# qwerty35/lsc_dr_planner

Hardware: AMD Instinct MI355X
Metric: qp_solves_per_sec (higher is better)
Workload: dtype f64; 1 GPU; configs[1]: 64 agents x M=5 x ~20 LSC half-spaces/seg, fp64 -- 64 agents/GPU x M=5 segments x 20 LSC neighbours (dim=3, forest swarm after 3 warm-up replans), fp64: dual active-set phase (one workgroup per QP) with the batched PDIP behind it for what it leaves; batch_seed=1000, precision=f64, row_format=f64, collective_backend=none (single process), agents_per_gpu=64, agents_total=64, ranks=1, distinct_devices=1, launch=single process, segments=5, lsc_neighbours=20, dim=3, rows_per_qp=1074, allgather=False, pipeline=False, hip_graph=False

## Files before the change

lsc_dr_planner_amd/csrc/lscqp_das_body.inc:

```
#if LSCQP_DAS_PROLOGUE
#define DAS_CLS(f) ka_##f
#else
#define DAS_CLS(f) cls.f
#endif
    const int tid = threadIdx.x, lane = tid & 63, wv = tid >> 6;
#ifdef LSCQP_DAS_LAYOUT
    constexpr Layout L = LSCQP_DAS_LAYOUT;
#else
    const Layout L = Layout::make(M, dim, kmax, cacheC, stage_rows);
#endif
    DAS_T_DECL();
    const int P = L.P, NX = L.NX, NPAIR = L.NPAIR;
    const int kcap = L.kmax;
    double* const H_ = smem + L.o_hdr;
    double* const sfc_ = smem + L.o_sfc;
    double* const c_ = smem + L.o_c;
    double* const cu_ = smem + L.o_cu;
    double* const lam_ = smem + L.o_lam;
    double* const plo_ = smem + L.o_plo;
    double* const phi_ = smem + L.o_phi;
    int* const pix_ = reinterpret_cast<int*>(smem + L.o_pix);
    double* const W_ = smem + L.o_W;
    double* const Jm_ = smem + L.o_L;
    double* const u_ = smem + L.o_u;
// ... 81 lines not shown
    int2 pwr[kPB];
#pragma unroll
    for (int u = 0; u < kPB; u++) pwr[u] = pairs_g[min(tid + u * T, NPAIR - 1)];
    {
        const double* hsrc = reinterpret_cast<const double*>(hdr + q);
        const double* ssrc = reinterpret_cast<const double*>(sfc) + q * 6 * M;
        for (int e = tid; e < 32 + (cls.use_sfc ? 6 * M : 0); e += T) (e < 32 ? H_[e] : sfc_[e - 32]) = e < 32 ? hsrc[e] : ssrc[e - 32];
        if (tid >= 64 - 36 && tid < 64) dq_[tid - (64 - 36)] = tab[(size_t)M * table_stride(M) + (tid - (64 - 36))];
        if (tid < 6) {
            const double w = tid == 0 ? cls.world_min[0] : tid == 1 ? cls.world_min[1] : tid == 2 ? cls.world_min[2] : tid == 3 ? cls.world_max[0] : tid == 4 ? cls.world_max[1] : cls.world_max[2];
            wb_[tid] = w;
        }
    }
    __syncthreads();
#endif
    DAS_T(0);
    const lscqp_header* Hd = reinterpret_cast<const lscqp_header*>(H_);
    const lscqp_box* sfcl = reinterpret_cast<const lscqp_box*>(sfc_);
#if !LSCQP_DAS_PROLOGUE
    const int n_obs = Hd->n_obs;
#endif
    auto hand_over = [&](int steps, int why) {
        for (int e = tid; e < NX; e += T) x_out[q * NX + e] = x_init ? x_init[q * NX + e] : Hd->p0[fdiv(e, 1.0f / (float)P)];
        if (tid == 0) {
            obj_out[q] = 0.0;
            status_out[q] = LSCQP_STATUS_ITER_LIMIT;
            if (info_out) {
                info_out[q].iterations = 0;
                info_out[q].flags = 0;
                info_out[q].res_primal = 0.0;
                info_out[q].res_dual = (double)why;
                info_out[q].gap = (double)steps;
            }
        }
    };
    auto infeasible_out = [&](int steps, double violation) {
        for (int e = tid; e < NX; e += T) x_out[q * NX + e] = x_init ? x_init[q * NX + e] : Hd->p0[fdiv(e, 1.0f / (float)P)];
        if (tid == 0) {
            obj_out[q] = 0.0;
            status_out[q] = LSCQP_STATUS_INFEASIBLE;
            if (info_out) {
                info_out[q].iterations = steps;
                info_out[q].flags = LSCQP_INFO_ACTIVE_SET;
                info_out[q].res_primal = violation;
                info_out[q].res_dual = 0.0;
                info_out[q].gap = 0.0;
            }
        }
    };
#if LSCQP_DAS_PROLOGUE
    if (!in_cap)
#else
    if (n_obs > cap || n_obs < 0)
#endif
    {
        hand_over(0, LSCQP_DAS_WHY_CAPACITY);
        LSCQP_DAS_END(kDasHandedOver);
    }
    const double dt = DAS_CLS(dt);
    const double org0 = Hd->p0[0], org1 = Hd->p0[1], org2 = Hd->p0[2];
    const double* const org = Hd->p0;
    int ts = Hd->terminal_segments;
    if (ts <= 0) {
        const double g0 = Hd->goal[0] - org0, g1 = Hd->goal[1] - org1, g2 = Hd->goal[2] - org2;
        ts = (int)((M * dt - sqrt(g0 * g0 + g1 * g1 + g2 * g2) / Hd->nominal_velocity + 1e-9) / dt);
        if (ts < 1) ts = 1;
    }
    if (ts > M) ts = M;
    const double q2s = DAS_CLS(q2s), wt2 = 2.0 * DAS_CLS(w_t);
    const double* const tb = tab + (size_t)(ts - 1) * table_stride(M);
    const double* const U1 = tb, * const U2 = tb + P, * const G1 = tb + 2 * P, * const Cg = tb + 3 * P;
    const bool comm_on = DAS_CLS(comm_range) > 0;
    const double rho_pair = 0.5 * DAS_CLS(comm_range) - Hd->radius;
    const double rho_wp = 0.5 * DAS_CLS(comm_range) - 1e-5;
#if !LSCQP_DAS_PROLOGUE
    const int nL = n_obs * P;
#endif
    const float iP = 1.0f / (float)P;
    const bool staged = stage_rows > 0 && nL <= stage_rows;
    bool rows_in_lds = false;

#if LSCQP_DAS_PROLOGUE
    constexpr int NE = 4;
    double tu1[NE], tu2[NE], tg1[NE];
#pragma unroll
    for (int i = 0; i < NE; i++) {
        const int e = tid + i * T < NX ? tid + i * T : 0;
        const int cp = e - P * fdiv(e, iP);
        tu1[i] = U1[cp], tu2[i] = U2[cp], tg1[i] = G1[cp];
    }
#else
    auto fetch_row = [&](int j, double& x, double& y, double& z, double& w) {
        if constexpr (F32) {
            const float4 f = reinterpret_cast<const float4*>(rows)[roff + (uint64_t)j];
            x = f.x, y = f.y, z = f.z, w = f.w;
        } else {
            const double4 d = *reinterpret_cast<const double4*>(&rows[roff + (uint64_t)j]);
            x = d.x, y = d.y, z = d.z, w = d.w;
        }
    };
    constexpr int NE = 4;
    double tu1[NE], tu2[NE], tg1[NE];
#pragma unroll
    for (int i = 0; i < NE; i++) {
        const int e = tid + i * T;
        if (e < NX) {
            const int cp = e - P * fdiv(e, iP);
            tu1[i] = U1[cp], tu2[i] = U2[cp], tg1[i] = G1[cp];
        }
    }
    double px[kU], py[kU], pz[kU], pw[kU];
#pragma unroll
    for (int u = 0; u < kU; u++) px[u] = py[u] = pz[u] = 0.0, pw[u] = -1.0;
    if (nL > 0) {
#pragma unroll
        for (int u = 0; u < kU; u++) {
            const int j = tid + u * T;
            fetch_row(j < nL ? j : 0, px[u], py[u], pz[u], pw[u]);
        }
    }
#endif

    constexpr int kCPre = (NW == 4 && !PEEL && !SCREEN) ? 6 : 0;
    double cpre[kCPre > 0 ? kCPre : 1];
#if LSCQP_DAS_PROLOGUE
    const bool c_fits = kCPre > 0 && P * P <= kCPre * T;
    const bool c_prefetched = c_fits && cacheC;
#else
    const bool c_prefetched = kCPre > 0 && cacheC && P * P <= kCPre * T;
    const bool c_fits = c_prefetched;
#endif
    if constexpr (kCPre > 0) {
        if (c_fits) {
#pragma unroll
            for (int i = 0; i < kCPre; i++) {
                const int e = tid + i * T;
                cpre[i] = Cg[e < P * P ? e : 0];
            }
        }
    }
#if LSCQP_DAS_STEP_PATH & 2
#ifndef LSCQP_DAS_LAYOUT
#error "LSCQP_DAS_STEP_PATH & 2 needs the compile-time carve"
#endif
    static_assert(NW > 1, "the first pass's barrier publishes the table");
    constexpr bool kTableEarly = kCPre > 0 && L.P * L.P <= kCPre * T;
    static_assert(!kTableEarly || LSCQP_DAS_PROLOGUE, "the table is stored from cpre[]: it needs the prologue that always loads it");
#else
    constexpr bool kTableEarly = false;
#endif

    bool empty = false;
    const double hv_c = dt * 0.2, ha_c = dt * dt * 0.05;
    for (int r0 = tid; r0 < NPAIR; r0 += kPB * T) {
        if (r0 != tid) {
#pragma unroll
            for (int u = 0; u < kPB; u++) pwr[u] = pairs_g[min(r0 + u * T, NPAIR - 1)];
        }
#pragma unroll
        for (int u = 0; u < kPB; u++) {
            if ((r0 - tid) + u * T >= NPAIR) break;
            const int r = r0 + u * T;
            const int w0 = pwr[u].x, w1 = pwr[u].y;
            const int fam = w1 & 3, k = (w1 >> 2) & 3, m = (w1 >> 4) & 15;
            const bool last = (w1 >> 8) & 1, rs = (w1 >> 9) & 1;
            const double ok_ = org[k], wlo = wb_[k], whi = wb_[3 + k], wpk = Hd->next_waypoint[k] - ok_;
            const double hv = Hd->vmax[k] * hv_c, ha = Hd->amax[k] * ha_c;
            double lo = wlo - ok_, hi = whi - ok_;
            if (DAS_CLS(rsfc) && rs) {
                lo = -100.0 - ok_;
                hi = 100.0 - ok_;
            }
            if (DAS_CLS(use_sfc)) {
                lo = fmax(lo, sfcl[m].bmin[k] - ok_);
                hi = fmin(hi, sfcl[m].bmax[k] - ok_);
            }
            const double clo = fmax(lo, fmax(-rho_pair, wpk - rho_wp)), chi = fmin(hi, fmin(rho_pair, wpk + rho_wp));
            lo = (comm_on && last) ? clo : lo;
            hi = (comm_on && last) ? chi : hi;
            const double hs = fam == 1 ? hv : fam == 2 ? ha : rho_pair;
            lo = fam == 0 ? lo : -hs;
            hi = fam == 0 ? hi : hs;
            if (r < NPAIR) {
                if (fam == 0 && (w0 >> 24) != 0 && lo > hi) empty = true;
                plo_[r] = lo, phi_[r] = hi;
                pix_[r] = w0;
            }
        }
    }
#pragma unroll
    for (int i = 0; i < NE; i++) {
        const int e = tid + i * T;
        if (e < NX) {
            const int k = fdiv(e, iP), cp = e - k * P;
            const double c1 = Hd->v0[k] * dt * 0.2;
            const double c2 = Hd->a0[k] * dt * dt * 0.05 + 2.0 * c1;
            const double fixv = (cp == 1) ? c1 : (cp == 2) ? c2 : 0.0;
            const double cv = fixv - c1 * tu1[i] - c2 * tu2[i] + wt2 * (Hd->goal[k] - org[k]) * tg1[i];
            c_[e] = cv;
            cu_[e] = cv;
        }
    }
    if (dim == 2)
        for (int e = tid; e < P; e += T) c_[2 * P + e] = 0.0;
#if LSCQP_DAS_STEP_PATH & 2
    {
        double2* const J2 = reinterpret_cast<double2*>(Jm_);
        for (int e = tid; e < kcap * LDL / 2; e += T) J2[e] = make_double2(0.0, 0.0);
    }
#endif
#if LSCQP_DAS_STEP_PATH & 8
    for (int e = tid; e < NX; e += T) lam_[e] = 0.0;
#endif
#if LSCQP_DAS_PROLOGUE
    const bool empty_w = __ballot(empty) != 0;
    if constexpr (NW > 1) {
        if (lane == 0) red_[20 + wv] = empty_w ? 1.0 : 0.0;
    }
    LSCQP_DAS_BARRIER();
    bool empty_g = empty_w;
    if constexpr (NW > 1) {
        empty_g = false;
#pragma unroll
        for (int w = 0; w < NW; w++) empty_g = empty_g || red_[20 + w] != 0.0;
    }
#else
    if (tid == 0) ctl_[4] = 0.0;
    LSCQP_DAS_BARRIER();
    if (empty) ctl_[4] = 1.0;
    LSCQP_DAS_BARRIER();
#endif
#if LSCQP_DAS_PROLOGUE
    if (empty_g)
#else
    if (ctl_[4] != 0.0)
#endif
    {
        double ov = 0.0;
        if (wv == 0) {
            for (int r = lane; r < NPAIR; r += 64)
                if ((pix_[r] >> 24) != 0) ov = fmax(ov, plo_[r] - phi_[r]);
            ov = wave_max(ov);
        }
        infeasible_out(0, ov);
        LSCQP_DAS_END(kDasInfeasible);
    }
    DAS_T(1);

    auto translate = [&](int j, double x, double y, double z, double w, double& nx, double& ny, double& nz, double& b) -> bool {
        nx = x, ny = y, nz = (dim == 3) ? z : 0.0;
        b = (dim == 3) ? w - (x * org0 + y * org1 + z * org2) : w - (x * org0 + y * org1 + 0.0);
        return !(x * x + y * y + z * z < 1e-10) && (j - P * fdiv(j, iP)) >= 3;
    };
    auto load_row = [&](int j, double& nx, double& ny, double& nz, double& b) -> bool {
        if (rows_in_lds) {
            nx = Sx_[j], ny = Sy_[j], nz = Sz_[j], b = Sb_[j];
            return b != -1.0 || nx != 0.0 || ny != 0.0 || nz != 0.0;
        }
        double x, y, z, w;
        fetch_row(j, x, y, z, w);
        return translate(j, x, y, z, w, nx, ny, nz, b);
    };
    auto pair_val = [&](int pk, const double* vec) -> double {
        const int type = pk >> 24, e0 = (pk >> 12) & 0xfff, e1 = pk & 0xfff;
        const int i0 = (type == 4) ? e1 : e0 + max(type - 1, 0);
        const int i1 = (type == 3) ? e0 + 1 : e0;
        const double a1 = (type <= 1) ? 0.0 : (type == 3) ? -2.0 : -1.0;
        const double a2 = (type == 3) ? 1.0 : 0.0;
        const double v0 = vec[i0], v1 = vec[i1], v2 = vec[e0];
        return (v0 + a1 * v1) + a2 * v2;
    };
    auto ent_of = [&](int e) -> int {
        const int k = fdiv(e, iP);
        return (k << 16) | (e - k * P);
    };
    auto decode = [&](int rid, Row& R) {
        R.ent[0] = R.ent[1] = R.ent[2] = 0;
        R.coef[0] = R.coef[1] = R.coef[2] = 0.0;
        if (rid < nL) {
            const int cp = rid - P * fdiv(rid, iP);
            double nx, ny, nz, b;
            (void)load_row(rid, nx, ny, nz, b);
            R.ent[0] = cp, R.ent[1] = (1 << 16) | cp, R.ent[2] = (2 << 16) | cp;
            R.coef[0] = nx, R.coef[1] = ny, R.coef[2] = (dim == 3) ? nz : 0.0;
            R.rhs = b;
            return;
        }
        const int s = rid - nL, r = s >> 1, pk = pix_[r];
        const int type = pk >> 24, e0 = (pk >> 12) & 0xfff, e1 = pk & 0xfff;
        const double sg = (s & 1) ? -1.0 : 1.0;
        R.rhs = (s & 1) ? -phi_[r] : plo_[r];
        const bool t1 = type == 1, t2 = type == 2, t3 = type == 3;
        R.ent[0] = ent_of(t1 ? e0 : t2 ? e0 + 1 : t3 ? e0 + 2 : e1);
        R.ent[1] = t1 ? 0 : ent_of(t3 ? e0 + 1 : e0);
        R.ent[2] = t3 ? ent_of(e0) : 0;
        R.coef[0] = sg;
        R.coef[1] = t1 ? 0.0 : t3 ? -2.0 * sg : -sg;
        R.coef[2] = t3 ? sg : 0.0;
    };
    auto row_dot = [&](const int* ent, const double* coef, const double* vec) -> double {
        return coef[0] * vec[ent_axis(ent[0]) * P + ent_cp(ent[0])] + coef[1] * vec[ent_axis(ent[1]) * P + ent_cp(ent[1])] +
               coef[2] * vec[ent_axis(ent[2]) * P + ent_cp(ent[2])];
    };

    bool first_pass = true;
    auto pass_local = [&](double& bv, int& bi) {
        bv = 1e300;
        bi = 0x7fffffff;
        auto see = [&](double slack, int id) {
            slack = (slack == slack) ? slack : -1e308;
            const bool lt = slack < bv;
            bv = lt ? slack : bv;
            bi = lt ? id : bi;
        };
        auto eval = [&](int j0, const double* rx, const double* ry, const double* rz, const double* rb) {
#pragma unroll
            for (int u = 0; u < kU; u++) {
                const int j = j0 + u * T, jc = j < nL ? j : 0;
                const int cp = jc - P * fdiv(jc, iP);
                see(rx[u] * c_[cp] + ry[u] * c_[P + cp] + rz[u] * c_[2 * P + cp] - rb[u], j);
            }
        };
        auto prep = [&](int j0, const double* x, const double* y, const double* z, const double* w, double* rx, double* ry, double* rz, double* rb) {
#pragma unroll
            for (int u = 0; u < kU; u++) {
                const int j = j0 + u * T, jc = j < nL ? j : 0;
                const bool ok = translate(jc, x[u], y[u], z[u], w[u], rx[u], ry[u], rz[u], rb[u]) && j < nL;
                rx[u] = ok ? rx[u] : 0.0, ry[u] = ok ? ry[u] : 0.0, rz[u] = ok ? rz[u] : 0.0, rb[u] = ok ? rb[u] : -1.0;
            }
        };
        auto stage = [&](int j0, const double* rx, const double* ry, const double* rz, const double* rb) {
#pragma unroll
            for (int u = 0; u < kU; u++) {
                const int j = j0 + u * T;
                if (j < nL) Sx_[j] = rx[u], Sy_[j] = ry[u], Sz_[j] = rz[u], Sb_[j] = rb[u];
            }
        };
        double rx[kU], ry[kU], rz[kU], rb[kU];
        if (first_pass) {
            prep(tid, px, py, pz, pw, rx, ry, rz, rb);
            if (staged) stage(tid, rx, ry, rz, rb);
            eval(tid, rx, ry, rz, rb);
            for (int j0 = tid + kU * T; kMaxNL > kU * T && j0 < nL; j0 += kU * T) {
                double x[kU], y[kU], z[kU], w[kU];
#pragma unroll
                for (int u = 0; u < kU; u++) fetch_row(j0 + u * T < nL ? j0 + u * T : 0, x[u], y[u], z[u], w[u]);
                prep(j0, x, y, z, w, rx, ry, rz, rb);
                if (staged) stage(j0, rx, ry, rz, rb);
                eval(j0, rx, ry, rz, rb);
            }
        } else if (rows_in_lds) {
#if LSCQP_DAS_STEP_PATH & 1
            for (int j0 = tid; j0 < nL; j0 += kU * T) {
                double lx[kU], ly[kU], lz[kU], lb[kU];
#pragma unroll
                for (int u = 0; u < kU; u++) {
                    const int j = j0 + u * T, jc = j < nL ? j : 0;
                    lx[u] = Sx_[jc], ly[u] = Sy_[jc], lz[u] = Sz_[jc], lb[u] = Sb_[jc];
                }
#pragma unroll
                for (int u = 0; u < kU; u++) {
                    const bool in = j0 + u * T < nL;
                    rx[u] = in ? lx[u] : 0.0, ry[u] = in ? ly[u] : 0.0, rz[u] = in ? lz[u] : 0.0, rb[u] = in ? lb[u] : -1.0;
                }
                eval(j0, rx, ry, rz, rb);
            }
#else
            for (int j0 = tid; j0 < nL; j0 += kU * T) {
#pragma unroll
                for (int u = 0; u < kU; u++) {
                    const int j = j0 + u * T, jc = j < nL ? j : 0;
                    rx[u] = Sx_[jc], ry[u] = Sy_[jc], rz[u] = Sz_[jc], rb[u] = (j < nL) ? Sb_[jc] : 1e300;
                    if (!(j < nL)) rx[u] = ry[u] = rz[u] = 0.0, rb[u] = -1.0;
                }
                eval(j0, rx, ry, rz, rb);
            }
#endif
        } else {
            for (int j0 = tid; j0 < nL; j0 += kU * T) {
                double x[kU], y[kU], z[kU], w[kU];
#pragma unroll
                for (int u = 0; u < kU; u++) fetch_row(j0 + u * T < nL ? j0 + u * T : 0, x[u], y[u], z[u], w[u]);
                prep(j0, x, y, z, w, rx, ry, rz, rb);
                eval(j0, rx, ry, rz, rb);
            }
        }
        first_pass = false;
        DAS_T(8);
        for (int r0 = tid; r0 < NPAIR; r0 += 2 * T) {
            const int r1 = r0 + T, r1c = r1 < NPAIR ? r1 : r0;
            const int pk0 = pix_[r0], pk1 = pix_[r1c];
            const double lo0 = plo_[r0], hi0 = phi_[r0], lo1 = plo_[r1c], hi1 = phi_[r1c];
            const double d0 = pair_val(pk0, c_), d1 = pair_val(pk1, c_);
            const bool on0 = (pk0 >> 24) != 0, on1 = (pk1 >> 24) != 0 && r1 < NPAIR;
            see(on0 ? d0 - lo0 : 1.0, nL + 2 * r0);
            see(on0 ? hi0 - d0 : 1.0, nL + 2 * r0 + 1);
            see(on1 ? d1 - lo1 : 1.0, nL + 2 * r1);
            see(on1 ? hi1 - d1 : 1.0, nL + 2 * r1 + 1);
        }
        DAS_T(9);
    };
    auto pass_combine = [&](const double* rb_, double& bv, int& bi) {
        bv = rb_[0], bi = reinterpret_cast<const int*>(rb_ + 4)[0];
#pragma unroll
        for (int w = 1; w < NW; w++) {
            const double ov = rb_[w];
            const int oi = reinterpret_cast<const int*>(rb_ + 4)[w];
            if (ov < bv || (ov == bv && oi < bi)) bv = ov, bi = oi;
        }
    };
    auto pass = [&](double& best, int& bid) {
        const bool was_first = first_pass;
        double bv;
        int bi;
        pass_local(bv, bi);
#if LSCQP_DAS_STEP_PATH & 2
        if constexpr (kTableEarly) {
            if (was_first) {
#pragma unroll
                for (int i = 0; i < kCPre; i++) {
                    const int e = tid + i * T;
                    if (e < P * P) Cc_[e] = cpre[i];
                }
            }
        }
#endif
        wave_argmin(bv, bi);
        if constexpr (NW > 1) {
            double* const rb_ = red_ + 24 * par;
            par ^= 1;
            if (lane == 0) {
                rb_[wv] = bv;
                reinterpret_cast<int*>(rb_ + 4)[wv] = bi;
            }
            LSCQP_DAS_BARRIER();
            pass_combine(rb_, bv, bi);
        } else if (staged && was_first) {
            LSCQP_DAS_BARRIER();
        }
        if (staged) rows_in_lds = true;
        best = bv, bid = bi;
    };

    const double* Cm = kTableEarly ? Cc_ : Cg;
    auto factor_remove = [&](int k_, int l_) -> bool {
        bool ok = true;
        if (wv == 0) {
            const int k = __builtin_amdgcn_readfirstlane(k_), l = __builtin_amdgcn_readfirstlane(l_);
            const bool mine = lane < k;
            const int c = mine ? lane : 0;
            const int cn = c - (c > l ? 1 : 0);
            double carry = Jm_[l * LDL + c];
            double a = Jm_[l * LDL + l];
            for (int j = l; j < k - 1; j++) {
                const double x = Jm_[(j + 1) * LDL + c];
                const double b = Jm_[(j + 1) * LDL + l];
                const double r2 = a * a + b * b;
                if (!(r2 > 1e-280)) ok = false;
                const double ir = rsqrt(fmax(r2, 1e-300));
                const double ca = a * ir, sb = b * ir;
                const double fin = ca * x - sb * carry;
                carry = ca * carry + sb * x;
                a = r2 * ir;
                if (mine && lane != l) Jm_[j * LDL + cn] = fin;
            }
            if (mine) Jm_[(k - 1) * LDL + lane] = 0.0, Jm_[lane * LDL + k - 1] = 0.0;
            LSCQP_DAS_WAVE_SYNC();
        }
        return ok;
    };
    auto solve_factor = [&](int k_, double vi, double* yy) -> double {
        const int k = __builtin_amdgcn_readfirstlane(k_);
        const bool mine = lane < k;
        const int ll = min(lane, kcap - 1);
        vi = mine ? vi : 0.0;
        double yi = 0.0, ri = 0.0;
        for (int j0 = 0; j0 < k; j0 += 8) {
            double Jr[8];
#pragma unroll
            for (int t_ = 0; t_ < 8; t_++) Jr[t_] = Jm_[ll * LDL + min(j0 + t_, kcap)];
#pragma unroll
            for (int t_ = 0; t_ < 8; t_++) yi += Jr[t_] * lscqp::bcast(vi, j0 + t_);
        }
        yi = mine ? yi : 0.0;
        if (yy) *yy = wave_sum(yi * yi);
        for (int j0 = 0; j0 < k; j0 += 8) {
            double Jc[8];
#pragma unroll
            for (int t_ = 0; t_ < 8; t_++) Jc[t_] = Jm_[min(j0 + t_, kcap - 1) * LDL + ll];
#pragma unroll
            for (int t_ = 0; t_ < 8; t_++) ri += Jc[t_] * lscqp::bcast(yi, j0 + t_);
        }
        ri = mine ? ri : 0.0;
        if (lane < kcap + 4) r_[lane] = ri;
        return ri;
    };
    auto add_columns = [&](int k, const double* wts, const double* base) {
        for (int e = tid; e < NX; e += T) {
            double a = base ? base[e] : c_[e];
            for (int j = 0; j < k; j++) a += wts[j] * W_[(size_t)j * NX + e];
            c_[e] = a;
        }
    };

    const int NZA = 3 * (M - 1) + (es ? 1 : 3);
    auto finish_local = [&](int k, double& rd, double& gs, double& part) {
#if LSCQP_DAS_PROLOGUE
        const double dt = wb_[6], q2s = wb_[7], ka_w_t = ctl_[4], ka_w_c = red_[44], wt2 = 2.0 * ka_w_t;
#endif
#if LSCQP_DAS_STEP_PATH & 8
#if !LSCQP_DAS_PROLOGUE
#error "LSCQP_DAS_STEP_PATH & 8 reads the class's scalars from LDS: it needs the rescheduled prologue"
#endif
        static_assert(NW > 1, "the stationarity rows take one trip of the workgroup");
        auto objective_local = [&]() {
#if LSCQP_DAS_STEP_PATH & 32
            static_assert(NW > 1, "the objective's lanes are the second wavefront's");
            part = 0.0;
            if (__builtin_amdgcn_readfirstlane(wv) == 1) {
                const bool on = lane < dim * M;
                const int lv = on ? lane : dim * M - 1;
                const int kx = lv / M, m = lv - kx * M;
                const double* cc = &c_[kx * P + 6 * m];
                double cv[6], dqv[36];
                double ok_ = org[kx], gl_ = Hd->goal[kx];
#pragma unroll
                for (int i = 0; i < 6; i++) cv[i] = cc[i];
#pragma unroll
                for (int i = 0; i < 36; i++) dqv[i] = dq_[i];
                asm volatile("" : "+v"(ok_), "+v"(gl_));
#pragma unroll
                for (int i = 0; i < 6; i++) asm volatile("" : "+v"(cv[i]));
#pragma unroll
                for (int i = 0; i < 36; i++) asm volatile("" : "+v"(dqv[i]));
                const double j0 = (cv[3] - cv[0]) - 3.0 * (cv[2] - cv[1]);
                const double j1 = (cv[4] - cv[1]) - 3.0 * (cv[3] - cv[2]);
                const double j2 = (cv[5] - cv[2]) - 3.0 * (cv[4] - cv[3]);
                const double quad = 0.2 * (j0 * j0 + j2 * j2) + (2.0 / 15.0) * j1 * j1 + 0.2 * (j0 * j1 + j1 * j2) + (1.0 / 15.0) * j0 * j2;
                double pp = 0.5 * q2s * 3600.0 * quad;
                double corr = 0;
                const double s0 = cv[0] + ok_, s1 = cv[1] + ok_, s2 = cv[2] + ok_, s3 = cv[3] + ok_, s4 = cv[4] + ok_, s5 = cv[5] + ok_;
#pragma unroll
                for (int i = 0; i < 6; i++) {
                    const double* dr = dqv + 6 * i;
                    double r = 0;
                    r += dr[0] * s0, r += dr[1] * s1, r += dr[2] * s2, r += dr[3] * s3, r += dr[4] * s4, r += dr[5] * s5;
                    corr += r * (cv[i] + ok_);
                }
                pp += DAS_CLS(w_c) * corr;
                const double dgoal = cv[5] - (gl_ - ok_);
                pp += (m >= M - ts) ? DAS_CLS(w_t) * dgoal * dgoal : 0.0;
                const double sum = part + pp;
                part = on ? sum : part;
            }
#else
            part = 0.0;
            for (int lv = tid - (NW > 1 ? 64 : 0); lv < dim * M; lv += T) {
                if (lv < 0) continue;
                const int kx = lv / M, m = lv - kx * M;
                const double* cc = &c_[kx * P + 6 * m];
                const double j0 = (cc[3] - cc[0]) - 3.0 * (cc[2] - cc[1]);
                const double j1 = (cc[4] - cc[1]) - 3.0 * (cc[3] - cc[2]);
// ... 182 lines not shown
        for (int w = 1; w < NW; w++) rd = fmax(rd, rb_[8 + w]), gs = fmax(gs, rb_[12 + w]), part += rb_[16 + w];
    };
    auto finish_verdict = [&](double rd, double gs, double part, double& res_d, double& obj) {
        res_d = (part == part && fabs(part) < 1e300) ? rd / fmax(1.0, gs) : 1e300;
        obj = part;
    };
    auto finish = [&](int k, double& res_d, double& obj) {
        double rd, gs, part;
        finish_local(k, rd, gs, part);
        lscqp::wave_reduce3<lscqp::OpMax, lscqp::OpMax, lscqp::OpSum>(rd, gs, part);
        if constexpr (NW > 1) {
            double* const rb_ = red_ + 24 * par;
            par ^= 1;
            if (lane == 0) rb_[8 + wv] = rd, rb_[12 + wv] = gs, rb_[16 + wv] = part;
            LSCQP_DAS_BARRIER();
            finish_combine(rb_, rd, gs, part);
        }
        finish_verdict(rd, gs, part, res_d, obj);
    };

    int k = 0, steps = 0, why = LSCQP_DAS_WHY_VERIFICATION;
    bool polished = false, solved = false, haveC = false, haveJ = false, proven = false;
    double res_p = 0.0, res_d = 0.0, obj = 0.0;
    auto write_out = [&]() {
        for (int e = tid; e < NX; e += T) x_out[q * NX + e] = c_[e] + org[fdiv(e, iP)];
        if (tid == 0) {
            obj_out[q] = obj;
            status_out[q] = LSCQP_STATUS_OPTIMAL;
            if (info_out) {
                info_out[q].iterations = steps;
                info_out[q].flags = LSCQP_INFO_ACTIVE_SET;
                info_out[q].res_primal = res_p;
                info_out[q].res_dual = res_d;
                info_out[q].gap = 0.0;
            }
        }
    };
    double best;
    int bid;
    bool peeled = false;
    if constexpr (PEEL || SCREEN) {
        pass(best, bid);
        DAS_T(2);
        if (!(best < -kTolP)) {
            res_p = fmax(0.0, -best);
            finish(0, res_d, obj);
            DAS_T(4);
            if (res_d <= kTolD) write_out();
            else hand_over(0, LSCQP_DAS_WHY_VERIFICATION);
            DAS_T(7);
            DAS_T_FLUSH();
            LSCQP_DAS_END(res_d <= kTolD ? kDasSolved : kDasHandedOver);
        }
        peeled = true;
    }
    for (;;) {
        if (!((PEEL || SCREEN) && peeled)) {
            pass(best, bid);
            DAS_T(steps == 0 ? 2 : 3);
        }
        peeled = false;
        if (!(best < -kTolP)) {
            res_p = fmax(0.0, -best);
            finish(k, res_d, obj);
            DAS_T(4);
            if (res_d <= kTolD) {
                solved = true;
                break;
            }
            if (polished || k == 0) break;
#if LSCQP_DAS_STEP_PATH & 8
            if (tid == 0) {
                for (int j_ = 0; j_ < k; j_++)
#pragma unroll
                    for (int t_ = 0; t_ < 3; t_++) {
                        const int en = aint_[4 * j_ + 1 + t_], at = ent_axis(en) * P + ent_cp(en);
                        if (at < NX) lam_[at] = 0.0;
                    }
            }
#endif
            LSCQP_DAS_BARRIER();
            add_columns(k, u_, cu_);
            LSCQP_DAS_BARRIER();
            if (wv == 0) {
                const double rho = (lane < k) ? arhs_[lane] - row_dot(&aint_[4 * lane + 1], &acoef_[3 * lane], c_) : 0.0;
                const double du = solve_factor(k, rho, nullptr);
                const double un = (lane < k) ? u_[lane] + du : 0.0;
                const double umax = wave_max(fabs(un));
                const double neg = wave_max((lane < k && un < -1e-12 * umax) ? 1.0 : 0.0);
                if (lane < k) u_[lane] = fmax(un, 0.0);
                if (lane == 0) ctl_[7] = neg;
            }
            LSCQP_DAS_BARRIER();
            if (ctl_[7] != 0.0) {
                why = LSCQP_DAS_WHY_MULTIPLIER;
                break;
            }
            add_columns(k, r_, nullptr);
            LSCQP_DAS_BARRIER();
            polished = true;
            continue;
        }
        polished = false;
        if constexpr (SCREEN) break;
        if (k >= kmax) {
            why = LSCQP_DAS_WHY_ROWS;
            break;
        }
#if LSCQP_DAS_STEP_PATH & 2
        (void)haveJ, (void)haveC;
#else
        if (!haveJ) {
            if (wv == 0)
                for (int e = lane; e < kcap * LDL; e += 64) Jm_[e] = 0.0;
            haveJ = true;
        }
#endif
        if (!kTableEarly && cacheC && !haveC) {
            bool copied = false;
            if constexpr (kCPre > 0) {
                if (c_prefetched) {
#pragma unroll
                    for (int i = 0; i < kCPre; i++) {
                        const int e = tid + i * T;
                        if (e < P * P) Cc_[e] = cpre[i];
                    }
                    copied = true;
                }
            }
            if (!copied)
                for (int e = tid; e < P * P; e += T) Cc_[e] = Cg[e];
            haveC = true;
            Cm = Cc_;
            LSCQP_DAS_BARRIER();
        }
        Row Rp;
        decode(bid, Rp);
        if (tid == 0) {
            aint_[4 * kcap] = bid;
            for (int t = 0; t < 3; t++) aint_[4 * kcap + 1 + t] = Rp.ent[t], acoef_[3 * kcap + t] = Rp.coef[t];
            arhs_[kcap] = Rp.rhs;
            ctl_[3] = 0.0;
        }
        auto compute_wp = [&](int first_thread, int n_threads) {
            for (int e = tid - first_thread; e < NX; e += n_threads) {
                if (e < 0) continue;
                const int kx = fdiv(e, iP), cp = e - kx * P;
                W_[(size_t)k * NX + e] = ccol(Rp.ent, Rp.coef, kx, cp, Cm, P);
            }
        };
        if constexpr (NW == 1) compute_wp(0, T);
        DAS_T(5);
        double spp = 0.0;
        bool stop = false, first_step = true;
        for (;;) {
            steps++;
            if (steps > max_steps) {
                stop = true;
                why = LSCQP_DAS_WHY_STEPS;
                break;
            }
            if (NW > 1 && first_step && wv != 0) compute_wp(64, T - 64);
            if (wv == 0 && __builtin_amdgcn_readfirstlane(k) == 0) {
                if (first_step) spp = cdot(Rp.ent, Rp.coef, Rp.ent, Rp.coef, Cm, P);
                const double sp = row_dot(Rp.ent, Rp.coef, c_) - Rp.rhs;
                const double t = (spp > 1e-12 * spp) ? -sp / spp : 1e300;
                const int kind = (t < 1e299) ? 1 : 0;
                if (lane == 0) {
                    if (kind == 1) Jm_[0] = rsqrt(spp), u_[0] = ctl_[3] + t;
                    ctl_[0] = t;
                    ctl_[1] = (double)kind;
                    ctl_[2] = 0.0;
                    ctl_[3] += t;
                    ctl_[5] = (t < 1e299) ? 1.0 : 0.0;
                }
            } else if (wv == 0) {
                if (first_step) spp = cdot(Rp.ent, Rp.coef, Rp.ent, Rp.coef, Cm, P);
                const double vj = (lane < k) ? row_dot(Rp.ent, Rp.coef, W_ + (size_t)lane * NX) : 0.0;
                DAS_T(13);
                double yy;
                const double ri = solve_factor(k, vj, &yy);
                DAS_T(14);
                const double curv = spp - yy;
                const double sp = row_dot(Rp.ent, Rp.coef, c_) - Rp.rhs;
                const double t2 = (curv > 1e-12 * spp) ? -sp / curv : 1e300;
                double t1 = (lane < k && ri > 0.0) ? u_[lane] / ri : 1e300;
                int l = lane;
                wave_argmin(t1, l);
                const double t = fmin(t1, t2);
                int kind;
                if (!(t < 1e299)) kind = (sp < -1e-6) ? 3 : 0;
                else if (t2 <= t1) kind = 1;
                else kind = 2;
                DAS_T(15);
                if (kind == 1 || kind == 2) {
                    if (lane < k) u_[lane] = fmax(0.0, u_[lane] - t * ri);
                    if (kind == 1) {
                        const double idl = rsqrt(curv);
                        if (lane < k) Jm_[k * LDL + lane] = -ri * idl, Jm_[lane * LDL + k] = 0.0;
                        if (lane == 0) Jm_[k * LDL + k] = idl, u_[k] = ctl_[3] + t;
                    }
                }
                if (lane == 0) {
                    ctl_[0] = t;
                    ctl_[1] = (double)kind;
                    ctl_[2] = (double)l;
                    ctl_[3] += t;
                    ctl_[5] = (t2 < 1e299) ? 1.0 : 0.0;
                    ctl_[7] = -sp;
                }
            }
            first_step = false;
            DAS_T(10);
            LSCQP_DAS_BARRIER();
            const double t = ctl_[0];
            const int kind = __builtin_amdgcn_readfirstlane((int)ctl_[1]), l = __builtin_amdgcn_readfirstlane((int)ctl_[2]);
            if (kind == 0 || kind == 3) {
                stop = true;
                why = LSCQP_DAS_WHY_NO_STEP;
                proven = kind == 3;
                break;
            }
            const int ks = __builtin_amdgcn_readfirstlane(k);
            const bool primal = __builtin_amdgcn_readfirstlane((int)ctl_[5]) != 0;
            for (int e = tid; e < NX; e += T) {
                if (primal) {
                    double a = W_[(size_t)ks * NX + e];
                    for (int j0 = 0; j0 < ks; j0 += 4) {
                        double wj[4], rj[4];
#pragma unroll
                        for (int t_ = 0; t_ < 4; t_++)
                            wj[t_] = W_[(size_t)min(j0 + t_, ks) * NX + e], rj[t_] = r_[j0 + t_];
#pragma unroll
                        for (int t_ = 0; t_ < 4; t_++) a -= rj[t_] * wj[t_];
                    }
                    c_[e] += t * a;
                }
                if (kind == 2) {
                    double nxt = W_[(size_t)(l + 1) * NX + e];
                    for (int j = l; j < ks; j++) {
                        const double cur = nxt;
                        nxt = W_[(size_t)min(j + 2, ks) * NX + e];
                        W_[(size_t)j * NX + e] = cur;
                    }
                }
            }
            DAS_T(11);
            if (kind == 1) {
#if LSCQP_DAS_STEP_PATH & 4
                if (tid == 0) {
                    aint_[4 * k] = bid;
#pragma unroll
                    for (int t_ = 0; t_ < 3; t_++) aint_[4 * k + 1 + t_] = Rp.ent[t_], acoef_[3 * k + t_] = Rp.coef[t_];
                    arhs_[k] = Rp.rhs;
                }
#else
                if (tid == 0) {
                    for (int t_ = 0; t_ < 4; t_++) aint_[4 * k + t_] = aint_[4 * kcap + t_];
                    for (int t_ = 0; t_ < 3; t_++) acoef_[3 * k + t_] = acoef_[3 * kcap + t_];
                    arhs_[k] = arhs_[kcap];
                }
#endif
                k++;
                LSCQP_DAS_BARRIER();
                break;
            }
            if (wv == 0) {
                const bool mv = lane >= l && lane + 1 < k;
                const int from = mv ? lane + 1 : 0;
                int ai[4];
                double ac[3];
#pragma unroll
                for (int t_ = 0; t_ < 4; t_++) ai[t_] = aint_[4 * from + t_];
#pragma unroll
                for (int t_ = 0; t_ < 3; t_++) ac[t_] = acoef_[3 * from + t_];
                const double ah = arhs_[from], uu = u_[from];
                LSCQP_DAS_WAVE_SYNC();
                if (mv) {
#pragma unroll
                    for (int t_ = 0; t_ < 4; t_++) aint_[4 * lane + t_] = ai[t_];
#pragma unroll
                    for (int t_ = 0; t_ < 3; t_++) acoef_[3 * lane + t_] = ac[t_];
                    arhs_[lane] = ah, u_[lane] = uu;
                }
            }
            const bool okf = factor_remove(k, l);
            k--;
            if (wv == 0 && lane == 0) ctl_[6] = okf ? 0.0 : 1.0;
            LSCQP_DAS_BARRIER();
            DAS_T(12);
            if (ctl_[6] != 0.0) {
                stop = true;
                why = LSCQP_DAS_WHY_PIVOT;
                break;
            }
        }
        DAS_T(6);
        if (stop) break;
    }
    if (!solved) {
        if (proven) {
            const int* const pe = &aint_[4 * kcap + 1];
            const double* const pc = &acoef_[3 * kcap];
            double vr = 0.0;
            for (int j = 0; j < k; j++) vr += r_[j] * row_dot(pe, pc, W_ + (size_t)j * NX);
            const double spp = cdot(pe, pc, pe, pc, Cm, P);
            const double d0 = wb_[3] - wb_[0], d1 = wb_[4] - wb_[1], d2 = wb_[5] - wb_[2];
            const double reach = sqrt(fmax(spp - vr, 0.0) / spp * (pc[0] * pc[0] + pc[1] * pc[1] + pc[2] * pc[2]) * (d0 * d0 + d1 * d1 + d2 * d2));
            proven = ctl_[7] > 1e-6 + reach;
        }
        if (proven) infeasible_out(steps, ctl_[7]);
        else hand_over(steps, why);
        DAS_T_FLUSH();
        LSCQP_DAS_END(proven ? kDasInfeasible : kDasHandedOver);
    }

    write_out();
    DAS_T(7);
    DAS_T_FLUSH();
    LSCQP_DAS_END(kDasSolved);
#undef DAS_CLS
```

lsc_dr_planner_amd/csrc/lscqp_fused.hip:

```cpp
#include <atomic>

#include "lscqp_kernel.hpp"
#include "lscqp_launch.hpp"
#define LSCQP_DAS_CYCLES das_fused_cycles
#include "lscqp_das.hpp"

#define LSCQP_FCAT_(a, b, c, d, e, f) a##b##_##c##_##d##_##e##_##f
#define LSCQP_FCAT(a, b, c, d, e, f) LSCQP_FCAT_(a, b, c, d, e, f)
#define LSCQP_FUSED_FN LSCQP_FCAT(lscqp_launch_fused_, LSCQP_M, LSCQP_DIM, LSCQP_ES, LSCQP_NSLOT, LSCQP_W)

namespace lscqp_das {

constexpr bool carve_fits(int M, int dim, int kmax, int stage_rows) {
    return sizeof(double) * (size_t)Layout::make(M, dim, kmax, 1, stage_rows).total <= lscqp::kMaxLdsBytes;
}
#if LSCQP_M == 10 && LSCQP_DIM == 3
#define LSCQP_FUSED_PROLOGUE 0
#else
#define LSCQP_FUSED_PROLOGUE 1
#endif
#ifndef LSCQP_FUSED_STEP_PATH
#if LSCQP_M == 5 || (LSCQP_M == 10 && LSCQP_DIM == 2)
#define LSCQP_FUSED_STEP_PATH (7 | 8 | 32)
#else
#define LSCQP_FUSED_STEP_PATH 0
#endif
#endif
template <int M, int DIM, bool ES, int NSLOT, int W>
struct FusedCarve {
    static constexpr int kStage = lscqp::Cfg<M, DIM, ES, NSLOT, W, (int)sizeof(double)>::MAX_OBS * 6 * M;
    static constexpr int KMAX = carve_fits(M, DIM, kMaxK, kStage) ? kMaxK : 20;
    static_assert(carve_fits(M, DIM, KMAX, kStage), "the fused phase's carve does not fit the CU's LDS");
};

template <int M, int DIM, bool ES, int NSLOT, int W>
__global__ __launch_bounds__(256, 1) void das_pdip_kernel(DevClass cls, int cap, int kmax, int max_steps, int cacheC, int stage_rows,
                                                          const double* __restrict__ tab, int64_t n, const lscqp_header* __restrict__ hdr,
                                                          const lscqp_row* __restrict__ rows, const uint64_t* __restrict__ row_offsets,
                                                          const lscqp_box* __restrict__ sfc, const double* __restrict__ x_init,
                                                          double* __restrict__ x_out, double* __restrict__ obj_out, int32_t* __restrict__ status_out,
                                                          lscqp_info* __restrict__ info_out) {
    static_assert(W >= 1 && W <= 4, "the interior-point instance runs on the first W of the workgroup's four wavefronts");
    extern __shared__ __attribute__((aligned(16))) double smem[];
#if LSCQP_FUSED_PROLOGUE
    LSCQP_DAS_KERNARGS();
    const int64_t k0 = blockIdx.x;
    if (k0 >= n) return;
    const int64_t q = ka_order ? (int64_t)ka_order[k0] : k0;
#else
    const int64_t k0 = blockIdx.x;
    if (k0 >= n) return;
    const int64_t q = cls.order ? (int64_t)cls.order[k0] : k0;
#endif
    int verdict = kDasSolved;
    {
        using FC = FusedCarve<M, DIM, ES, NSLOT, W>;
        constexpr int NW = 4, T = 64 * NW;
#ifdef LSCQP_FUSED_ROW_SLOTS
        constexpr int kU = LSCQP_FUSED_ROW_SLOTS;
#else
        constexpr int kU = (FC::kStage + T - 1) / T < 4 ? (FC::kStage + T - 1) / T : 4;
#endif
        constexpr bool F32 = false, SCREEN = false, PEEL = false;
        constexpr int dim = DIM, es = ES ? 1 : 0, behind = 0;
        constexpr int kMaxNL = FC::kStage;
        static_assert(kU == 4 || kMaxNL <= kU * T, "the row slots must cover the carve's staged rows");
        static_assert(kU >= 1, "an instance has rows");
#define LSCQP_DAS_END(verdict_)   \
    do {                          \
        verdict = (verdict_);     \
        goto phase_done;          \
    } while (0)
#define LSCQP_DAS_LAYOUT Layout::make(M, DIM, FC::KMAX, 1, FC::kStage)
#define LSCQP_DAS_PROLOGUE LSCQP_FUSED_PROLOGUE
#define LSCQP_DAS_STEP_PATH LSCQP_FUSED_STEP_PATH
#include "lscqp_das_body.inc"
#undef LSCQP_DAS_STEP_PATH
#undef LSCQP_DAS_PROLOGUE
#undef LSCQP_DAS_LAYOUT
#undef LSCQP_DAS_END
    }
phase_done:
    verdict = __builtin_amdgcn_readfirstlane(verdict);
    if (verdict != kDasHandedOver) return;
    __syncthreads();
    if constexpr (W < 4) {
        if (__builtin_amdgcn_readfirstlane((int)(threadIdx.x >> 6)) >= W) return;
    }
    lscqp::lscqp_pdip_one<M, DIM, ES, NSLOT, W, double>(cls, q, smem, hdr, rows, row_offsets, sfc, x_init, x_out, obj_out, status_out, info_out);
}

}

extern "C" hipError_t LSCQP_FUSED_FN(const lscqp::DevClass* cls, int cap, int kmax, int max_steps, int cacheC, int stage_rows, const double* d_tab,
                                     int64_t n, const lscqp_header* hdr, const lscqp_row* rows, const uint64_t* row_offsets, const lscqp_box* sfc,
                                     const double* x_init, double* x_out, double* obj_out, int32_t* status_out, lscqp_info* info_out,
                                     hipStream_t stream) {
    using C = lscqp::Cfg<LSCQP_M, LSCQP_DIM, (LSCQP_ES != 0), LSCQP_NSLOT, LSCQP_W, (int)sizeof(double)>;
    using FC = lscqp_das::FusedCarve<LSCQP_M, LSCQP_DIM, (LSCQP_ES != 0), LSCQP_NSLOT, LSCQP_W>;
    auto kern = lscqp_das::das_pdip_kernel<LSCQP_M, LSCQP_DIM, (LSCQP_ES != 0), LSCQP_NSLOT, LSCQP_W>;
    if (kmax < 1 || kmax > lscqp_das::kMaxK || cls->rows_f32 || cls->queue || cls->scan || cls->repair != 3) return hipErrorInvalidValue;
    if (cls->n_obs_max > C::MAX_OBS || cap > C::MAX_OBS) return hipErrorNotSupported;
    if (kmax > FC::KMAX || stage_rows > FC::kStage) return hipErrorNotSupported;
    const size_t lds_das = sizeof(double) * (size_t)lscqp_das::Layout::make(LSCQP_M, LSCQP_DIM, FC::KMAX, 1, FC::kStage).total;
    const size_t lds = lds_das > C::lds_bytes() ? lds_das : C::lds_bytes();
    if (lds > lscqp::kMaxLdsBytes) return hipErrorNotSupported;
    static std::atomic<bool> attr_set[64];
    int dev = 0;
    if (hipGetDevice(&dev) != hipSuccess || dev < 0 || dev >= 64) return hipErrorInvalidDevice;
    if (!attr_set[dev].load(std::memory_order_acquire)) {
        const hipError_t e = hipFuncSetAttribute(reinterpret_cast<const void*>(kern), hipFuncAttributeMaxDynamicSharedMemorySize, (int)lscqp::kMaxLdsBytes);
        if (e != hipSuccess) return e;
        attr_set[dev].store(true, std::memory_order_release);
    }
    if (n <= 0) return hipSuccess;
    hipLaunchKernelGGL(kern, dim3((unsigned)n), dim3(256), lds, stream, *cls, cap, kmax, max_steps, cacheC, stage_rows, d_tab, n, hdr, rows, row_offsets, sfc,
                       x_init, x_out, obj_out, status_out, info_out);
    return hipGetLastError();
}

#ifdef LSCQP_DAS_TIMING
extern "C" int lscqp_das_fused_cycles(unsigned long long* out, int reset) {
    (void)hipMemcpyFromSymbol(out, HIP_SYMBOL(lscqp_das::das_fused_cycles), sizeof(unsigned long long) * 16);
    if (reset) {
        unsigned long long z[16] = {0};
        (void)hipMemcpyToSymbol(HIP_SYMBOL(lscqp_das::das_fused_cycles), z, sizeof z);
    }
    return 0;
}
#endif
```

Before: 7.263 million QP/s.

## Enable six micro-optimisations in fused DAS step path for M=5

Turns on six new step-path flags for the M=5 fused kernel. They keep per-thread copies of the two-sided pair rows in registers so the pricing pass skips re-reading LDS, and issue the single-block LSC row loads and the pair loads together ahead of the evaluation. They also vectorise the reads of the ballot and reduction slots as double2/int4, keep the running step sum u in a register instead of re-reading ctl_[3], and clamp pair indices before loading. These changes target LDS latency and instruction count in the hot pricing and step loops, at the cost of more register pressure.

```diff
diff --git a/lsc_dr_planner_amd/csrc/lscqp_das_body.inc b/lsc_dr_planner_amd/csrc/lscqp_das_body.inc
--- a/lsc_dr_planner_amd/csrc/lscqp_das_body.inc
+++ b/lsc_dr_planner_amd/csrc/lscqp_das_body.inc
@@ -257,6 +257,18 @@
 
     bool empty = false;
     const double hv_c = dt * 0.2, ha_c = dt * dt * 0.05;
+#if LSCQP_DAS_STEP_PATH & 2048
+#ifndef LSCQP_DAS_LAYOUT
+#error "LSCQP_DAS_STEP_PATH & 2048 sizes its register copy from the compile-time carve"
+#endif
+    constexpr int kPR = (L.NPAIR + T - 1) / T;
+    static_assert(kPR <= kPB && L.NPAIR <= kPB * T, "the section's first block of four slots holds every two-sided row of the shape");
+    int tp_pk[kPR], tp_i0[kPR], tp_i1[kPR], tp_e0[kPR];
+    double tp_a1[kPR], tp_a2[kPR], tp_lo[kPR], tp_hi[kPR];
+#pragma unroll
+    for (int u = 0; u < kPR; u++)
+        tp_pk[u] = tp_i0[u] = tp_i1[u] = tp_e0[u] = 0, tp_a1[u] = tp_a2[u] = tp_lo[u] = tp_hi[u] = 0.0;
+#endif
     for (int r0 = tid; r0 < NPAIR; r0 += kPB * T) {
         if (r0 != tid) {
 #pragma unroll
@@ -291,6 +303,20 @@
                 plo_[r] = lo, phi_[r] = hi;
                 pix_[r] = w0;
             }
+#if LSCQP_DAS_STEP_PATH & 2048
+            if (u < kPR) {
+                const int pk = r < NPAIR ? w0 : 0;
+                const int type = pk >> 24, e0 = (pk >> 12) & 0xfff, e1 = pk & 0xfff;
+                const int us = u < kPR ? u : 0;
+                tp_pk[us] = pk;
+                tp_i0[us] = (type == 4) ? e1 : e0 + max(type - 1, 0);
+                tp_i1[us] = (type == 3) ? e0 + 1 : e0;
+                tp_e0[us] = e0;
+                tp_a1[us] = (type <= 1) ? 0.0 : (type == 3) ? -2.0 : -1.0;
+                tp_a2[us] = (type == 3) ? 1.0 : 0.0;
+                tp_lo[us] = lo, tp_hi[us] = hi;
+            }
+#endif
         }
     }
 #pragma unroll
@@ -325,9 +351,15 @@
     LSCQP_DAS_BARRIER();
     bool empty_g = empty_w;
     if constexpr (NW > 1) {
+#if LSCQP_DAS_STEP_PATH & 64
+        static_assert(NW == 4 && L.o_red % 2 == 0, "four ballots, two 16-byte words");
+        const double2 b01 = *reinterpret_cast<const double2*>(red_ + 20), b23 = *reinterpret_cast<const double2*>(red_ + 22);
+        empty_g = fmax(fmax(b01.x, b01.y), fmax(b23.x, b23.y)) != 0.0;
+#else
         empty_g = false;
 #pragma unroll
         for (int w = 0; w < NW; w++) empty_g = empty_g || red_[20 + w] != 0.0;
+#endif
     }
 #else
     if (tid == 0) ctl_[4] = 0.0;
@@ -391,10 +423,20 @@
             R.rhs = b;
             return;
         }
+#if LSCQP_DAS_STEP_PATH & 512
+        const int s = rid - nL, rc_ = min(s >> 1, NPAIR - 1);
+        const int pk = pix_[rc_];
+        const double lo_w = plo_[rc_], hi_w = phi_[rc_];
+#else
         const int s = rid - nL, r = s >> 1, pk = pix_[r];
+#endif
         const int type = pk >> 24, e0 = (pk >> 12) & 0xfff, e1 = pk & 0xfff;
         const double sg = (s & 1) ? -1.0 : 1.0;
+#if LSCQP_DAS_STEP_PATH & 512
+        R.rhs = (s & 1) ? -hi_w : lo_w;
+#else
         R.rhs = (s & 1) ? -phi_[r] : plo_[r];
+#endif
         const bool t1 = type == 1, t2 = type == 2, t3 = type == 3;
         R.ent[0] = ent_of(t1 ? e0 : t2 ? e0 + 1 : t3 ? e0 + 2 : e1);
         R.ent[1] = t1 ? 0 : ent_of(t3 ? e0 + 1 : e0);
@@ -442,6 +484,25 @@
             }
         };
         double rx[kU], ry[kU], rz[kU], rb[kU];
+#if LSCQP_DAS_STEP_PATH & 2048
+        double tv0[kPR], tv1[kPR], tv2[kPR];
+        bool ts_asked = false;
+        auto ts_request = [&]() {
+#pragma unroll
+            for (int u = 0; u < kPR; u++) tv0[u] = c_[tp_i0[u]], tv1[u] = c_[tp_i1[u]], tv2[u] = c_[tp_e0[u]];
+            ts_asked = true;
+        };
+        auto ts_see = [&]() {
+#pragma unroll
+            for (int u = 0; u < kPR; u++) {
+                const int r = tid + u * T;
+                const double d = (tv0[u] + tp_a1[u] * tv1[u]) + tp_a2[u] * tv2[u];
+                const bool on = (tp_pk[u] >> 24) != 0;
+                see(on ? d - tp_lo[u] : 1.0, nL + 2 * r);
+                see(on ? tp_hi[u] - d : 1.0, nL + 2 * r + 1);
+            }
+        };
+#endif
         if (first_pass) {
             prep(tid, px, py, pz, pw, rx, ry, rz, rb);
             if (staged) stage(tid, rx, ry, rz, rb);
@@ -455,7 +516,30 @@
                 eval(j0, rx, ry, rz, rb);
             }
         } else if (rows_in_lds) {
-#if LSCQP_DAS_STEP_PATH & 1
+#if LSCQP_DAS_STEP_PATH & 2048
+            static_assert((LSCQP_DAS_STEP_PATH & 1) && kMaxNL <= kU * T, "one block of clamped, untested loads covers the instance's rows");
+            double lx[kU], ly[kU], lz[kU], lb[kU], cx[kU], cy[kU], cz[kU];
+#pragma unroll
+            for (int u = 0; u < kU; u++) {
+                const int j = tid + u * T, jc = j < nL ? j : 0;
+                lx[u] = Sx_[jc], ly[u] = Sy_[jc], lz[u] = Sz_[jc], lb[u] = Sb_[jc];
+            }
+#pragma unroll
+            for (int u = 0; u < kU; u++) {
+                const int j = tid + u * T, jc = j < nL ? j : 0;
+                const int cp = jc - P * fdiv(jc, iP);
+                cx[u] = c_[cp], cy[u] = c_[P + cp], cz[u] = c_[2 * P + cp];
+            }
+            ts_request();
+            __builtin_amdgcn_sched_barrier(0);
+#pragma unroll
+            for (int u = 0; u < kU; u++) {
+                const int j = tid + u * T;
+                const bool in = j < nL;
+                rx[u] = in ? lx[u] : 0.0, ry[u] = in ? ly[u] : 0.0, rz[u] = in ? lz[u] : 0.0, rb[u] = in ? lb[u] : -1.0;
+                see(rx[u] * cx[u] + ry[u] * cy[u] + rz[u] * cz[u] - rb[u], j);
+            }
+#elif LSCQP_DAS_STEP_PATH & 1
             for (int j0 = tid; j0 < nL; j0 += kU * T) {
                 double lx[kU], ly[kU], lz[kU], lb[kU];
 #pragma unroll
@@ -492,6 +576,10 @@
         }
         first_pass = false;
         DAS_T(8);
+#if LSCQP_DAS_STEP_PATH & 2048
+        if (!ts_asked) ts_request();
+        ts_see();
+#else
         for (int r0 = tid; r0 < NPAIR; r0 += 2 * T) {
             const int r1 = r0 + T, r1c = r1 < NPAIR ? r1 : r0;
             const int pk0 = pix_[r0], pk1 = pix_[r1c];
@@ -503,9 +591,23 @@
             see(on1 ? d1 - lo1 : 1.0, nL + 2 * r1);
             see(on1 ? hi1 - d1 : 1.0, nL + 2 * r1 + 1);
         }
+#endif
         DAS_T(9);
     };
     auto pass_combine = [&](const double* rb_, double& bv, int& bi) {
+#if LSCQP_DAS_STEP_PATH & 128
+        static_assert(NW == 4 && L.o_red % 2 == 0, "four values and four ids, three 16-byte words");
+        const double2 v01 = *reinterpret_cast<const double2*>(rb_), v23 = *reinterpret_cast<const double2*>(rb_ + 2);
+        const int4 ids = *reinterpret_cast<const int4*>(rb_ + 4);
+        const double ovs[4] = {v01.x, v01.y, v23.x, v23.y};
+        const int ois[4] = {ids.x, ids.y, ids.z, ids.w};
+        bv = ovs[0], bi = ois[0];
+#pragma unroll
+        for (int w = 1; w < NW; w++) {
+            const bool lt = (ovs[w] < bv) | ((ovs[w] == bv) & (ois[w] < bi));
+            bv = lt ? ovs[w] : bv, bi = lt ? ois[w] : bi;
+        }
+#else
         bv = rb_[0], bi = reinterpret_cast<const int*>(rb_ + 4)[0];
 #pragma unroll
         for (int w = 1; w < NW; w++) {
@@ -513,6 +615,7 @@
             const int oi = reinterpret_cast<const int*>(rb_ + 4)[w];
             if (ov < bv || (ov == bv && oi < bi)) bv = ov, bi = oi;
         }
+#endif
     };
     auto pass = [&](double& best, int& bid) {
         const bool was_first = first_pass;
@@ -1001,6 +1104,12 @@
         if constexpr (NW == 1) compute_wp(0, T);
         DAS_T(5);
         double spp = 0.0;
+#if LSCQP_DAS_STEP_PATH & 1024
+        double u_cand = 0.0;
+#define DAS_U_CAND u_cand
+#else
+#define DAS_U_CAND ctl_[3]
+#endif
         bool stop = false, first_step = true;
         for (;;) {
             steps++;
@@ -1015,6 +1124,17 @@
                 const double sp = row_dot(Rp.ent, Rp.coef, c_) - Rp.rhs;
                 const double t = (spp > 1e-12 * spp) ? -sp / spp : 1e300;
                 const int kind = (t < 1e299) ? 1 : 0;
+#if LSCQP_DAS_STEP_PATH & 1024
+                u_cand = u_cand + t;
+                if (lane == 0) {
+                    if (kind == 1) Jm_[0] = rsqrt(spp), u_[0] = u_cand;
+                    ctl_[0] = t;
+                    ctl_[1] = (double)kind;
+                    ctl_[2] = 0.0;
+                    ctl_[3] = u_cand;
+                    ctl_[5] = (t < 1e299) ? 1.0 : 0.0;
+                }
+#else
                 if (lane == 0) {
                     if (kind == 1) Jm_[0] = rsqrt(spp), u_[0] = ctl_[3] + t;
                     ctl_[0] = t;
@@ -1023,6 +1143,7 @@
                     ctl_[3] += t;
                     ctl_[5] = (t < 1e299) ? 1.0 : 0.0;
                 }
+#endif
             } else if (wv == 0) {
                 if (first_step) spp = cdot(Rp.ent, Rp.coef, Rp.ent, Rp.coef, Cm, P);
                 const double vj = (lane < k) ? row_dot(Rp.ent, Rp.coef, W_ + (size_t)lane * NX) : 0.0;
@@ -1047,14 +1168,21 @@
                     if (kind == 1) {
                         const double idl = rsqrt(curv);
                         if (lane < k) Jm_[k * LDL + lane] = -ri * idl, Jm_[lane * LDL + k] = 0.0;
-                        if (lane == 0) Jm_[k * LDL + k] = idl, u_[k] = ctl_[3] + t;
+                        if (lane == 0) Jm_[k * LDL + k] = idl, u_[k] = DAS_U_CAND + t;
                     }
                 }
+#if LSCQP_DAS_STEP_PATH & 1024
+                u_cand = u_cand + t;
+#endif
                 if (lane == 0) {
                     ctl_[0] = t;
                     ctl_[1] = (double)kind;
                     ctl_[2] = (double)l;
+#if LSCQP_DAS_STEP_PATH & 1024
+                    ctl_[3] = u_cand;
+#else
                     ctl_[3] += t;
+#endif
                     ctl_[5] = (t2 < 1e299) ? 1.0 : 0.0;
                     ctl_[7] = -sp;
                 }
@@ -1064,6 +1192,10 @@
             LSCQP_DAS_BARRIER();
             const double t = ctl_[0];
             const int kind = __builtin_amdgcn_readfirstlane((int)ctl_[1]), l = __builtin_amdgcn_readfirstlane((int)ctl_[2]);
+#if LSCQP_DAS_STEP_PATH & 256
+            double primal_w = ctl_[5];
+            asm volatile("" : "+v"(primal_w));
+#endif
             if (kind == 0 || kind == 3) {
                 stop = true;
                 why = LSCQP_DAS_WHY_NO_STEP;
@@ -1071,7 +1203,11 @@
                 break;
             }
             const int ks = __builtin_amdgcn_readfirstlane(k);
+#if LSCQP_DAS_STEP_PATH & 256
+            const bool primal = __builtin_amdgcn_readfirstlane((int)primal_w) != 0;
+#else
             const bool primal = __builtin_amdgcn_readfirstlane((int)ctl_[5]) != 0;
+#endif
             for (int e = tid; e < NX; e += T) {
                 if (primal) {
                     double a = W_[(size_t)ks * NX + e];
@@ -1168,4 +1304,5 @@
     DAS_T(7);
     DAS_T_FLUSH();
     LSCQP_DAS_END(kDasSolved);
+#undef DAS_U_CAND
 #undef DAS_CLS
diff --git a/lsc_dr_planner_amd/csrc/lscqp_fused.hip b/lsc_dr_planner_amd/csrc/lscqp_fused.hip
--- a/lsc_dr_planner_amd/csrc/lscqp_fused.hip
+++ b/lsc_dr_planner_amd/csrc/lscqp_fused.hip
@@ -21,7 +21,7 @@
 #endif
 #ifndef LSCQP_FUSED_STEP_PATH
 #if LSCQP_M == 5 || (LSCQP_M == 10 && LSCQP_DIM == 2)
-#define LSCQP_FUSED_STEP_PATH (7 | 8 | 32)
+#define LSCQP_FUSED_STEP_PATH (7 | 8 | 32 | 64 | 128 | 256 | 512 | 1024 | 2048)
 #else
 #define LSCQP_FUSED_STEP_PATH 0
 #endif
```

New measurement: 7.618 million QP/s, median of 6. +4.9%, better.
